# hardcamls/video-coding

Measured on NVIDIA B200. Metric: decoded megapixels/sec (1920x1080 420 baseline), higher is better.
Workload: dtype u8/int16/int32 (integer, bit-exact)

## Files before the change

### video-coding_b200/csrc/hcj_common.h

```cpp
#pragma once
#include <stdint.h>

#define HCJ_LUT_BITS 10
#define HCJ_LUT_SIZE (1 << HCJ_LUT_BITS)
#define HCJ_LUT_NSUB 8
#define HCJ_LUT_SUB_BITS 6
#define HCJ_LUT_SUB_SIZE (1 << HCJ_LUT_SUB_BITS)
#define HCJ_LUT_ENTRIES (HCJ_LUT_SIZE + HCJ_LUT_NSUB * HCJ_LUT_SUB_SIZE)
#define HCJ_MAX_BPM 10
#define HCJ_MAX_COMP 4
#ifndef HCJ_IDCT_THREADS
#define HCJ_IDCT_THREADS 128
#endif
#ifndef HCJ_IDCT_CTAS_PER_SM
#define HCJ_IDCT_CTAS_PER_SM 5
#endif

#define HCJ_DEV_OK 0
#define HCJ_DEV_NO_DC_CODE (-2)
#define HCJ_DEV_NO_AC_CODE (-3)
#define HCJ_DEV_COEF_INDEX (-4)
#define HCJ_DEV_BITS_OOB (-9)
#define HCJ_DEV_NO_TERMINATOR (-20)
#define HCJ_DEV_RESTART_COUNT (-21)
#define HCJ_DEV_DC_RANGE (-23)

struct HcjTableMeta {
  uint32_t full_off;
  uint32_t max_bits;
};

struct HcjTableSet {
  HcjTableMeta meta[HCJ_MAX_COMP][2];
  uint32_t primary_off;
  uint32_t npairs;
};

struct HcjCompGeom {
  int32_t hs, vs;
  int32_t decoded_w, decoded_h;
  int32_t actual_w, actual_h;
  int32_t pair;
  int32_t qt;
  int32_t first_blk;
  uint8_t up_h, up_v;
  uint16_t pad_;
  uint64_t plane_off;
  uint64_t out_off;
};

struct HcjImageDesc {
  uint64_t file_off;
  uint32_t file_len;
  uint32_t scan_start;
  uint64_t ent_off;
  uint32_t ent_cap;
  uint32_t seg_off;
  uint32_t nseg_expected;
  uint32_t ri;
  int32_t ncomp, bpm;
  int32_t mcus_wide, mcus_high;
  uint32_t nmcu, nblocks;
  uint64_t coef_off;
  HcjCompGeom comp[HCJ_MAX_COMP];
  uint8_t blk_comp[HCJ_MAX_BPM + 2];
  uint8_t blk_bx[HCJ_MAX_BPM + 2];
  uint8_t blk_by[HCJ_MAX_BPM + 2];
  uint8_t wide_idct;
// ... 25 lines not shown
```

### video-coding_b200/csrc/hcj_device.cuh

```cuda
#pragma once
#include <stdint.h>

#include "hcj_common.h"

#if defined(__CUDACC__)
#define HCJ_HD __host__ __device__ __forceinline__
#else
#define HCJ_HD inline
#endif

namespace hcjdev {

HCJ_HD uint32_t bswap32(uint32_t x) {
#if defined(__CUDA_ARCH__)
  return __byte_perm(x, 0, 0x0123);
#else
  return (x >> 24) | ((x >> 8) & 0xff00u) | ((x << 8) & 0xff0000u) | (x << 24);
#endif
}

HCJ_HD uint32_t load_raw_word(const uint32_t *__restrict__ words, uint32_t idx, uint32_t end_bits) {
  if ((idx << 5) >= end_bits) return 0u;
#if defined(__CUDA_ARCH__)
  return __ldg(words + idx);
// ... 347 lines not shown
    }
  }
  if (err) *err_pos = br.pos;
  return err;
}

struct FastReader {
  const uint32_t *words;
  uint32_t pos, w0, w1, r0, r1;
  HCJ_HD static uint32_t ld(const uint32_t *p) {
#if defined(__CUDA_ARCH__)
    return __ldg(p);
#else
    return *p;
#endif
  }
  HCJ_HD void init(const uint32_t *words_, uint32_t pos_) {
    words = words_;
    pos = pos_;
    const uint32_t i = pos_ >> 5;
    w0 = bswap32(ld(words + i));
    w1 = bswap32(ld(words + i + 1));
    r0 = ld(words + i + 2);
    r1 = ld(words + i + 3);
  }
  HCJ_HD uint32_t window() const {
#if defined(__CUDA_ARCH__)
    return __funnelshift_l(w1, w0, pos);
#else
    uint32_t s = pos & 31u;
    return s ? (w0 << s) | (w1 >> (32u - s)) : w0;
#endif
  }
  HCJ_HD void consume(uint32_t n) {
    const uint32_t np = pos + n;
    const uint32_t cross = (np ^ pos) & 32u;
    pos = np;
    if (cross) {
      w0 = w1;
      w1 = bswap32(r0);
      r0 = r1;
    }
#if defined(__CUDA_ARCH__)
    asm volatile(
        "{\n\t.reg .pred p;\n\tsetp.ne.u32 p, %2, 0;\n\t@p ld.global.nc.L2::128B.u32 %0, [%1];\n\t}"
        : "+r"(r1)
        : "l"(words + (np >> 5) + 3), "r"(cross));
#else
    if (cross) r1 = ld(words + (np >> 5) + 3);
#endif
  }
};

HCJ_HD int32_t fast_value(uint32_t win, uint32_t len, uint32_t sh) {
  const uint32_t t = win << len;
  const uint32_t m = shr_clamp(t, sh), mask = shr_clamp(0xffffffffu, sh);
  return (int32_t)m - (int32_t)(mask & ~(uint32_t)((int32_t)t >> 31));
}

HCJ_HD bool z_block_done(uint32_t z) { return z >= 64u; }
HCJ_HD bool z_overrun(uint32_t z) { return z > 64u && z <= HCJ_ZADV_EOB; }
HCJ_HD bool z_no_code(uint32_t z) { return z >= 256u; }

struct ExactLane {
  FastReader br;
  uint32_t c, z;
  uint32_t tdc, tac, qoff;
  uint32_t comp;
  int32_t blk;
  int32_t pcur, p0, p1, p2, p3;
  uint32_t share, sumabs, qmax;
};

HCJ_HD void exact_bind_block(ExactLane &s, const FastTables T) {
  const BlkInfo bi = T.blkinfo[s.c];
  s.tdc = bi.tdc;
  s.tac = bi.tac;
  s.qoff = bi.qoff;
  s.comp = bi.comp_qmax & 0xffu;
  s.qmax = bi.comp_qmax >> 8;
  s.pcur = s.comp == 0u ? s.p0 : s.comp == 1u ? s.p1 : s.comp == 2u ? s.p2 : s.p3;
}
HCJ_HD void exact_save_pred(ExactLane &s) {
  s.p0 = s.comp == 0u ? s.pcur : s.p0;
  s.p1 = s.comp == 1u ? s.pcur : s.p1;
  s.p2 = s.comp == 2u ? s.pcur : s.p2;
  s.p3 = s.comp == 3u ? s.pcur : s.p3;
}
HCJ_HD void exact_next_block(ExactLane &s, const FastTables T, uint32_t bpm) {
  exact_save_pred(s);
  s.c = s.c + 1u == bpm ? 0u : s.c + 1u;
  s.z = 0u;
  s.share = 0u;
  s.sumabs = 0u;
  exact_bind_block(s, T);
}
HCJ_HD bool exact_share_may_be_wide(const ExactLane &s) {
  return s.sumabs >= 0x10000u || (uint64_t)s.share + (uint64_t)s.sumabs * s.qmax >= (uint64_t)HCJ_WIDE_SHARE;
}
HCJ_HD uint32_t exact_share(const ExactLane &s, const FastTables T, const int16_t *row) {
  uint64_t a = s.share;
  for (int zi = 1; zi < 64; zi++) {
    const int32_t v = row[zi];
    a += (uint64_t)(uint32_t)(v < 0 ? -v : v) * (uint32_t)T.quant[s.qoff + zi];
  }
  return a > 0xffffffffull ? 0xffffffffu : (uint32_t)a;
}

HCJ_HD void exact_ac_step(ExactLane &s, const FastTables T, int16_t *row) {
  const uint32_t win = s.br.window();
  const uint32_t e = fast_lookup(T, s.tac, win, false);
  const uint32_t znext = s.z + (e >> 24);
  const uint32_t sh = byte_of(e, 2);
  const int32_t v = fast_value(win, byte_of(e, 1), sh);
  if (sh != 32u && znext <= 64u) {
    row[znext - 1u] = (int16_t)v;
    s.sumabs += (uint32_t)(v < 0 ? -v : v);
  }
  s.br.consume(byte_of(e, 0));
  s.z = znext;
}
HCJ_HD void exact_ac_undo_no_code(ExactLane &s) { s.z -= 255u; }

HCJ_HD bool exact_dc_step(ExactLane &s, const FastTables T, int16_t *row) {
  const uint32_t win = s.br.window();
  const uint32_t e = fast_lookup(T, s.tdc, win, true);
  const int32_t pc = s.pcur + fast_value(win, byte_of(e, 1), byte_of(e, 2));
  if (e == HCJ_FAST_NONE || pc < -32768 || pc > 32767) return false;
  s.pcur = pc;
  s.blk++;
  row[0] = (int16_t)pc;
  s.share = (uint32_t)(pc < 0 ? -pc : pc) * (uint32_t)T.quant[s.qoff];
  s.sumabs = 0u;
  s.br.consume(byte_of(e, 0));
  s.z = 1u;
  return true;
}

HCJ_HD uint32_t multi_sync_entry(const uint32_t *fast_ac , uint32_t idx) {
  const uint32_t e = fast_ac[idx];
  if (e & HCJ_FAST_SLOW) return e;
  uint32_t pos = e & 0xffu, pre = 0, adv = e >> 24;
  while (adv != HCJ_ZADV_EOB && pos < (uint32_t)HCJ_LUT_BITS && pre + adv < 63u) {
    const uint32_t e2 = fast_ac[(idx << pos) & (HCJ_LUT_SIZE - 1)];
    if (e2 & HCJ_FAST_SLOW) break;
    if (pos + ((e2 >> 8) & 0xffu) > (uint32_t)HCJ_LUT_BITS) break;
    if (pos + (e2 & 0xffu) > 31u) break;
    pre += adv;
    adv = e2 >> 24;
    pos += e2 & 0xffu;
  }
  const uint32_t tot = pre + adv > 127u ? 127u : pre + adv;
  return pos | (pre << 8) | (tot << 24);
}

struct SyncLane {
  FastReader br;
  uint32_t c, z;
  uint32_t tdc, tac, comp;
  uint32_t nstart;
  int32_t d0, d1, d2, d3;
  uint32_t first_p, nbefore;
};
HCJ_HD void sync_bind_block(SyncLane &s, const FastTables T) {
  const BlkInfo bi = T.blkinfo[s.c];
  s.tdc = bi.tdc;
  s.tac = bi.tac;
  s.comp = bi.comp_qmax & 0xffu;
}
HCJ_HD void sync_next_block(SyncLane &s, const FastTables T, uint32_t bpm) {
  s.c = s.c + 1u == bpm ? 0u : s.c + 1u;
  s.z = 0u;
  sync_bind_block(s, T);
}
HCJ_HD void sync_ac_step_multi(SyncLane &s, const FastTables T, uint32_t lim_m) {
  const uint32_t win = s.br.window();
  const uint32_t idx = win >> (32 - HCJ_LUT_BITS);
// ... 132 lines not shown
  constexpr int t[64] = {0,  1,  8,  16, 9,  2,  3,  10, 17, 24, 32, 25, 18, 11, 4,  5,  12, 19, 26, 33, 40, 48,
                         41, 34, 27, 20, 13, 6,  7,  14, 21, 28, 35, 42, 49, 56, 57, 50, 43, 36, 29, 22, 15, 23,
                         30, 37, 44, 51, 58, 59, 52, 45, 38, 31, 39, 46, 53, 60, 61, 54, 47, 55, 62, 63};
  return t[i];
}
HCJ_HD constexpr int zigzag_forward(int i) {
  constexpr int t[64] = {0,  1,  5,  6,  14, 15, 27, 28, 2,  4,  7,  13, 16, 26, 29, 42, 3,  8,  12, 17, 25, 30,
                         41, 43, 9,  11, 18, 24, 31, 40, 44, 53, 10, 19, 23, 32, 39, 45, 52, 54, 20, 22, 33, 38,
                         46, 51, 55, 60, 21, 34, 37, 47, 50, 56, 59, 61, 35, 36, 48, 49, 57, 58, 62, 63};
  return t[i];
}

#define HCJ_QD(i, q) (((i) & 1) ? (int32_t)(q) << 8 : (int32_t)(q))
HCJ_HD int32_t dequant_lo(uint32_t cw, int32_t q) {
#if defined(__CUDA_ARCH__)
  int32_t d;
  asm("dp2a.lo.s32.u32 %0, %1, %2, %3;" : "=r"(d) : "r"(cw), "r"(q), "r"(0));
  return d;
#else
  return (int32_t)(int16_t)(cw & 0xffffu) * q;
#endif
}
HCJ_HD int32_t dequant_hi(uint32_t cw, int32_t q) {
#if defined(__CUDA_ARCH__)
  int32_t d;
  asm("dp2a.lo.s32.u32 %0, %1, %2, %3;" : "=r"(d) : "r"(cw), "r"(q), "r"(0));
  return d;
#else
  return (int32_t)(int16_t)(cw >> 16) * (q >> 8);
#endif
}

template <bool GUARD = true>
HCJ_HD bool reconstruct_fast(const uint32_t cw[32], const int32_t *__restrict__ qd , uint32_t out[16]) {
  int32_t v[64];
  uint32_t l1 = 0;
#pragma unroll
  for (int j = 0; j < 32; j++) {
    int32_t d0 = dequant_lo(cw[j], qd[2 * j]), d1 = dequant_hi(cw[j], qd[2 * j + 1]);
    v[zigzag_inverse(2 * j)] = d0;
    v[zigzag_inverse(2 * j + 1)] = d1;
    if (GUARD) l1 += (uint32_t)(d0 < 0 ? -d0 : d0) + (uint32_t)(d1 < 0 ? -d1 : d1);
  }
  if (GUARD && l1 >= (uint32_t)HCJ_IDCT_L1_LIMIT) return false;
  idct_8x8<int32_t, (128 << 14)>(v);
#pragma unroll
  for (int r = 0; r < 8; r++) {
    out[2 * r] = pack4_sat(v[8 * r], v[8 * r + 1], v[8 * r + 2], v[8 * r + 3]);
    out[2 * r + 1] = pack4_sat(v[8 * r + 4], v[8 * r + 5], v[8 * r + 6], v[8 * r + 7]);
  }
  return true;
}

HCJ_HD void reconstruct_wide(const uint32_t *cw, const int32_t *q, uint32_t *out) {
  int64_t w[64];
  for (int j = 0; j < 32; j++) {
    int64_t lo = (int16_t)(cw[j] & 0xffffu), hi = (int16_t)(cw[j] >> 16);
    w[zigzag_inverse(2 * j)] = lo * (int64_t)q[2 * j];
    w[zigzag_inverse(2 * j + 1)] = hi * (int64_t)q[2 * j + 1];
  }
  idct_8x8<int64_t>(w);
  for (int k = 0; k < 16; k++) {
    uint32_t word = 0;
    for (int i = 0; i < 4; i++) {
      int64_t sv = w[4 * k + i] < -128 ? -128 : w[4 * k + i] > 127 ? 127 : w[4 * k + i];
      word |= (uint32_t)(sv + 128) << (8 * i);
    }
    out[k] = word;
  }
}

HCJ_HD void reconstruct_block(const int16_t c[64], const uint16_t q[64], bool force_wide, uint8_t pix[64]) {
  uint32_t cw[32], out[16];
  int32_t q32[64], qd[64];
  for (int j = 0; j < 32; j++) cw[j] = (uint32_t)(uint16_t)c[2 * j] | ((uint32_t)(uint16_t)c[2 * j + 1] << 16);
  for (int i = 0; i < 64; i++) {
    q32[i] = q[i];
    qd[i] = HCJ_QD(i, q[i]);
  }
  if (force_wide || !reconstruct_fast<true>(cw, qd, out)) reconstruct_wide(cw, q32, out);
  for (int k = 0; k < 64; k++) pix[k] = (uint8_t)(out[k >> 2] >> (8 * (k & 3)));
}

template <typename T>
HCJ_HD T dequant_nat(const uint32_t cw[32], const int32_t *q, int n) {
  const int z = zigzag_forward(n);
  const int32_t c = (z & 1) ? (int32_t)(int16_t)(cw[z >> 1] >> 16) : (int32_t)(int16_t)(cw[z >> 1] & 0xffffu);
  return (T)c * (T)q[z];
}

template <typename T>
HCJ_HD void idct4_pass(T c0, T c1, T c2, T c3, T c5, T c6, T c7, int sh, T o[4]) {
  const T t0 = c0 * (T)(1 << 14);
  const T t2 = c2 * (T)15137 - c6 * (T)6270;
  const T t10 = t0 + t2, t12 = t0 - t2;
  const T a0 = c1 * (T)8697 - c3 * (T)17799 + c5 * (T)11893 - c7 * (T)1730;
  const T a2 = c1 * (T)20995 + c3 * (T)7373 - c5 * (T)4926 - c7 * (T)4176;
  const T r = (T)1 << (sh - 1);
  o[0] = (t10 + a2 + r) >> sh;
  o[1] = (t12 + a0 + r) >> sh;
  o[2] = (t12 - a0 + r) >> sh;
  o[3] = (t10 - a2 + r) >> sh;
}

template <typename T>
HCJ_HD void idct2_pass(T c0, T c1, T c3, T c5, T c7, int sh, T o[2]) {
// ... 362 lines not shown
```

### video-coding_b200/csrc/hcj_kernels.cu

```cuda
#include <cuda.h>
#include <cuda_runtime.h>
#include <stdint.h>
#include <stdlib.h>

#include "hcj_device.cuh"
#include "hcj_kernels.cuh"

namespace hcjk {

using namespace hcjdev;

constexpr int DS_THREADS = 256;
constexpr uint32_t DS_TILE = DS_THREADS * 16;

__device__ __forceinline__ uint32_t warp_incl_scan(uint32_t v, int lane) {
#pragma unroll
  for (int d = 1; d < 32; d <<= 1) {
    uint32_t t = __shfl_up_sync(0xffffffffu, v, d);
    if (lane >= d) v += t;
  }
  return v;
}

struct DsClass {
// ... 553 lines not shown
    sc.total_bits = total_bits;
    sc.bpm = d.bpm;
    sc.wide_flags = b.wide_flags;
    sc.blk_base = d.coef_off;
  }
  if (threadIdx.x < (uint32_t)d.ncomp) sc.tab[threadIdx.x] = tables_of(st, threadIdx.x);
}

__device__ __forceinline__ void raise_status(HcjImageState *st, int code, uint32_t bit_pos) {
  atomicMin(&st->err_key, ((unsigned long long)bit_pos << 8) | (unsigned long long)(-code));
}

constexpr int HR_ROW_WORDS = 36;
constexpr int HR_STAGE_WORDS = 32 * HR_ROW_WORDS;

struct PassIn {
  uint32_t p, cz, hi, end_bits;
  int32_t blk;
  int32_t pred[HCJ_MAX_COMP];
  int32_t nblocks_end;
  uint32_t share;
  bool valid;
};

__device__ __forceinline__ void warp_store_full(uint32_t mask, int32_t blk, uint32_t *stage, int lane, int16_t *coefs) {
  const int quarter = lane >> 3, sub = lane & 7;
#pragma unroll
  for (int p = 0; p < 8; p++) {
    if (((mask >> (4 * p)) & 0xfu) == 0u) continue;
    const int l = 4 * p + quarter;
    const int32_t bidx = __shfl_sync(0xffffffffu, blk, l);
    if ((mask >> l) & 1u) {
      uint4 *src = reinterpret_cast<uint4 *>(stage + l * HR_ROW_WORDS) + sub;
      const uint4 v = *src;
      *src = make_uint4(0u, 0u, 0u, 0u);
      reinterpret_cast<uint4 *>(coefs + (size_t)bidx * 64)[sub] = v;
    }
  }
}

__device__ __forceinline__ int warp_exact_fast(const ScanCtx &sc, const FastTables T, uint32_t *stage, int lane, PassIn &in,
                                               int16_t *coefs, uint32_t *err_pos) {
  const uint32_t bpm = sc.bpm;
  int16_t *row = reinterpret_cast<int16_t *>(stage + lane * HR_ROW_WORDS);
  const uint32_t lim = in.end_bits >= 32u ? in.end_bits - 32u : 0u;
  ExactLane s;
  s.c = in.cz >> 8;
  s.z = in.cz & 0xffu;
  s.blk = in.blk;
  s.p0 = in.pred[0], s.p1 = in.pred[1], s.p2 = in.pred[2], s.p3 = in.pred[3];
  s.share = in.share;
  s.sumabs = 0u;
  const bool entered = in.valid && in.p < lim;
  s.br.init(sc.words, entered ? in.p : 0u);
  exact_bind_block(s, T);
  int st = !entered ? 2 : s.z != 0u ? 0 : 1;
  int err = HCJ_DEV_OK;

  for (;;) {
    while (__any_sync(0xffffffffu, st == 0)) {
#pragma unroll
      for (int u = 0; u < 2; u++) {
        if (st == 0) {
          if (s.br.pos >= lim) {
            st = 2;
          } else {
            exact_ac_step(s, T, row);
            st = z_block_done(s.z) ? 1 : 0;
          }
        }
      }
    }
    if (!__any_sync(0xffffffffu, st == 1)) break;
    {
      if (st == 1 && s.z > 64u) {
        if (z_no_code(s.z)) {
          exact_ac_undo_no_code(s);
          st = 2;
        } else if (z_overrun(s.z)) {
          err = HCJ_DEV_COEF_INDEX;
          *err_pos = s.br.pos;
          st = 3;
        }
      }
      const bool have = st == 1 && s.z != 0u;
      if (have && exact_share_may_be_wide(s) && exact_share(s, T, row) >= (uint32_t)HCJ_WIDE_SHARE) flag_wide_block(sc, s.blk);
      warp_store_full(__ballot_sync(0xffffffffu, have), s.blk, stage, lane, coefs);
      if (have) exact_next_block(s, T, bpm);
      if (st == 1) {
        if (s.blk + 1 >= in.nblocks_end || s.br.pos >= lim || (s.c == 0u && s.br.pos >= in.hi)) st = 2;
        else st = exact_dc_step(s, T, row) ? 0 : 2;
      }
    }
  }
  if (entered && st == 2 && s.z != 0u) s.share = exact_share(s, T, row);
  if (entered) {
    exact_save_pred(s);
    in.p = s.br.pos;
    in.cz = (s.c << 8) | s.z;
    in.blk = s.blk;
    in.pred[0] = s.p0, in.pred[1] = s.p1, in.pred[2] = s.p2, in.pred[3] = s.p3;
    in.share = s.share;
    if (err) {
      in.valid = false;
      uint4 *src = reinterpret_cast<uint4 *>(row);
#pragma unroll
      for (int j = 0; j < 8; j++) src[j] = make_uint4(0u, 0u, 0u, 0u);
    }
  }
  return err;
}

__device__ __forceinline__ int warp_exact_pass(const ScanCtx &sc, const SmemTables &st, const Local L, uint32_t *stage,
                                               int lane, const PassIn &in, int16_t *coefs, uint32_t *err_pos) {
  uint32_t *coefs32 = reinterpret_cast<uint32_t *>(coefs);
  const uint32_t bpm = sc.bpm;
  uint32_t c = in.cz >> 8, z = in.cz & 0xffu, share = in.share;
  int32_t blk = in.blk;
  bool active = in.valid;
  uint32_t comp = st.blk_comp[c];
  Tables t = sc.tab[comp];
  const uint32_t stage_sa = (uint32_t)__cvta_generic_to_shared(stage);
  const uint32_t mine_sa = stage_sa + (uint32_t)lane * HR_ROW_WORDS * 4u;
  const uint32_t quant_sa = (uint32_t)__cvta_generic_to_shared(st.quant);
  uint32_t q_sa = quant_sa + comp * 512u;
  int32_t p0 = in.pred[0], p1 = in.pred[1], p2 = in.pred[2], p3 = in.pred[3];
  int32_t pcur = comp == 0u ? p0 : comp == 1u ? p1 : comp == 2u ? p2 : p3;
// ... 566 lines not shown
  fill_scan_ctx(sc, st, b, d, si.state->ent_len * 8u);
  __syncthreads();
  const Local LT{T, st.quant, st.blk_comp};
  int16_t *coefs = b.coefs + d.coef_off * 64;

  const uint32_t j = blockIdx.x * SPEC_WRITE_THREADS + threadIdx.x;
  PassIn in;
  in.valid = j < si.nsub;
  const uint32_t jj = in.valid ? j : 0u;
  const SpecSub q = spec_sub(si, jj);
  const uint32_t first = si.first[jj];
  in.valid = in.valid && (first >> 31) == 0u;
  in.p = q.lo + (first & 0xffffu);
  in.cz = 0u;
  const int4 dc = si.dc[jj], dpre = si.dpre[jj];
  in.pred[0] = dc.x + dpre.x, in.pred[1] = dc.y + dpre.y, in.pred[2] = dc.z + dpre.z, in.pred[3] = dc.w + dpre.w;
  in.blk = si.blk[jj] + (int32_t)((first >> 16) & 15u) - 1;
  in.hi = q.hi;
  in.end_bits = q.uend;
  in.nblocks_end = q.blk_end;
  in.share = 0;
  uint32_t err_pos = 0;
  int err = warp_exact_fast(sc, T, stage, lane, in, coefs, &err_pos);
  if (err) raise_status(si.state, err, err_pos);
  err = warp_exact_pass(sc, st, LT, stage, lane, in, coefs, &err_pos);
  if (err) raise_status(si.state, err, err_pos);
}

static inline size_t spec_base_smem(const DecodeBatchDev &b) {
  return ((sizeof(SmemTables) + 15) & ~size_t(15)) + ((sizeof(ScanCtx) + 15) & ~size_t(15)) + lut_smem_bytes(b);
}
void launch_huff_spec(const DecodeBatchDev &b, cudaStream_t s) {
  if (b.ls_hi <= b.ls_lo || b.max_sub_chunks == 0) return;
  const size_t base = spec_base_smem(b);
  const size_t smem_sync = base + multi_smem_bytes(b);
  const size_t smem_write = base + (SPEC_WRITE_THREADS / 32) * HR_STAGE_WORDS * sizeof(uint32_t);
  const dim3 grid(b.max_sub_chunks, b.ls_hi - b.ls_lo);
  if (b.spec_has_units) k_spec_units<<<b.ls_hi - b.ls_lo, SPEC_THREADS, 0, s>>>(b);
  k_spec_sync<<<grid, SPEC_THREADS, smem_sync, s>>>(b);
  k_spec_fix<<<b.ls_hi - b.ls_lo, SPEC_FIX_THREADS, base, s>>>(b);
  const dim3 grid_w((b.max_sub_chunks * SPEC_THREADS + SPEC_WRITE_THREADS - 1) / SPEC_WRITE_THREADS, b.ls_hi - b.ls_lo);
  k_spec_write<<<grid_w, SPEC_WRITE_THREADS, smem_write, s>>>(b);
}
int huff_spec_kernel_count(const DecodeBatchDev &b) { return 3 + (b.spec_has_units ? 1 : 0); }

constexpr int IDCT_MAX_THREADS = HCJ_IDCT_THREADS;

__device__ __forceinline__ void cp_async16(void *smem, const void *gmem) {
  uint32_t sa = (uint32_t)__cvta_generic_to_shared(smem);
  asm volatile("cp.async.cg.shared.global [%0], [%1], 16;\n" ::"r"(sa), "l"(gmem) : "memory");
}
__device__ __forceinline__ void cp_async_wait_all() { asm volatile("cp.async.wait_all;\n" ::: "memory"); }

__device__ __forceinline__ void store_block_rows(const uint32_t pix[16], uint8_t *dst, int stride, int x, int y,
                                                 int w_limit, int h_limit) {
  uint8_t *row = dst + (size_t)y * stride + x;
  const bool fast = (x + 8 <= w_limit) && (((uintptr_t)row & 7u) == 0) && ((stride & 7) == 0);
  if (fast) {
#pragma unroll
    for (int r = 0; r < 8; r++)
      if (y + r < h_limit) *reinterpret_cast<uint2 *>(row + (size_t)r * stride) = make_uint2(pix[2 * r], pix[2 * r + 1]);
  } else {
#pragma unroll
    for (int r = 0; r < 8; r++) {
      if (y + r >= h_limit) break;
#pragma unroll
      for (int i = 0; i < 8; i++)
        if (x + i < w_limit) row[(size_t)r * stride + i] = (uint8_t)(pix[2 * r + (i >> 2)] >> (8 * (i & 3)));
    }
  }
}

__device__ __noinline__ void wide_block_store(const uint32_t *cw, const int32_t *q, uint8_t *dst, int stride, int x, int y,
                                              int w_limit, int h_limit) {
  uint32_t pix[16];
  reconstruct_wide(cw, q, pix);
  store_block_rows(pix, dst, stride, x, y, w_limit, h_limit);
}

__device__ __noinline__ void wide_block_store_staged(const uint4 *tile, int slot, const int32_t *q, uint8_t *dst, int stride, int x,
                                                     int y, int w_limit, int h_limit) {
  uint32_t cw[32], pix[16];
  for (int j = 0; j < 8; j++) {
    const uint4 u = tile[slot * 8 + (j ^ (slot & 7))];
    cw[4 * j] = u.x, cw[4 * j + 1] = u.y, cw[4 * j + 2] = u.z, cw[4 * j + 3] = u.w;
  }
  reconstruct_wide(cw, q, pix);
  store_block_rows(pix, dst, stride, x, y, w_limit, h_limit);
}

template <int K>
__device__ __forceinline__ void store_block_rows_k(const uint32_t *pix, uint8_t *dst, int stride, int x, int y, int w_limit,
                                                   int h_limit) {
  uint8_t *row = dst + (size_t)y * stride + x;
  const bool fast = (x + K <= w_limit) && (((uintptr_t)row & (K - 1)) == 0) && ((stride & (K - 1)) == 0);
#pragma unroll
  for (int r = 0; r < K; r++) {
    if (y + r >= h_limit) break;
    uint8_t *p = row + (size_t)r * stride;
    if (fast) {
      if (K == 4) *reinterpret_cast<uint32_t *>(p) = pix[r];
      else if (K == 2) *reinterpret_cast<uint16_t *>(p) = (uint16_t)pix[r];
      else *p = (uint8_t)pix[r];
    } else {
#pragma unroll
      for (int i = 0; i < K; i++)
        if (x + i < w_limit) p[i] = (uint8_t)(pix[r] >> (8 * i));
    }
  }
}

template <int K>
__device__ __noinline__ void scaled_block_store_wide(const uint4 *tile, int slot, const int32_t *q, uint8_t *dst, int stride, int x,
                                                     int y, int h_limit) {
  uint32_t cw[32], pix[K];
  for (int j = 0; j < 8; j++) {
    const uint4 u = tile[slot * 8 + (j ^ (slot & 7))];
// ... 356 lines not shown
  const int tm = t.tm, vs_log = d.comp[0].vs == 2 ? 1 : 0;
  const int rows = 8 << vs_log, pitch_l = 16 * tm, pitch_c = 8 * tm;
  uint8_t *xcb = xch + rows * pitch_l, *xcr = xcb + 8 * pitch_c;
  const int x = (int)t.m0 * (int)((mp.misc >> 12) & 63u) + (int)(mp.xy & 0xffffu);
  const int y = (int)t.my * (int)((mp.misc >> 18) & 63u) + (int)(mp.xy >> 16);
  uint8_t *dst = c == 0 ? xch + (mp.xy >> 16) * pitch_l + (mp.xy & 0xffffu) : (c == 1 ? xcb : xcr) + (mp.xy & 0xffffu);
  const int pitch = c == 0 ? pitch_l : pitch_c;
  {
    uint32_t pix[16];
    reconstruct_fast<false>(cw, st.q + c * 128 + 64, pix);
    if (mine && !wide) {
#pragma unroll
      for (int r = 0; r < 8; r++) *reinterpret_cast<uint2 *>(dst + r * pitch) = make_uint2(pix[2 * r], pix[2 * r + 1]);
      if (c != 0) store_block_rows(pix, mp.plane, mp.stride, x, y, mp.stride, mp.h_limit);
    }
  }
  if (any_wide && wide) {
    const int16_t *cb = b.coefs + (t.blk0 + (uint64_t)slot) * 64;
    wide_block_to_xch(cb, st.q + c * 128, dst, pitch);
    if (c != 0) wide_block_store(reinterpret_cast<const uint32_t *>(cb), st.q + c * 128, mp.plane, mp.stride, x, y, mp.stride, mp.h_limit);
  }
  __syncthreads();
  const int width = d.width, height = d.height, cwid = d.comp[1].actual_w, chh = d.comp[1].actual_h;
  const int x_tile = (int)t.m0 * 16, y_tile = (int)t.my * rows, cx_tile = (int)t.m0 * 8, cy_tile = (int)t.my * 8;
  const bool right_deferred = cx_tile + 8 * tm < cwid;
  const bool bottom_deferred = vs_log && cy_tile + 8 < chh;
  uint8_t *out = b.out + d.out_off;
  uint8_t *plane_y = b.planes + d.comp[0].plane_off;
  const int stride_y = d.comp[0].decoded_w;
  const int nunits = rows * tm, nhalf = vs_log ? 8 * tm : nunits;
  const uint32_t recip = 65536u / (uint32_t)tm + 1u;
  for (int idx = tid; idx < nunits; idx += IDCT_MAX_THREADS) {
    const int k = idx < nhalf ? idx : idx - nhalf;
    const int rk = (int)(((uint32_t)k * recip) >> 16), m = k - rk * tm;
    const int r = vs_log ? 2 * rk + (idx < nhalf ? 0 : 1) : rk;
    const int px = x_tile + 16 * m, py = y_tile + r;
    if (py >= height || px >= width) continue;
    const uint4 vy = *reinterpret_cast<const uint4 *>(xch + r * pitch_l + 16 * m);
    if ((right_deferred && m == tm - 1) || (bottom_deferred && r == rows - 1)) {
      *reinterpret_cast<uint4 *>(plane_y + (size_t)py * stride_y + px) = vy;
      continue;
    }
    const int crow = r >> vs_log;
    const bool oy = vs_log && (r & 1);
    const int crow1 = (oy && cy_tile + crow + 1 <= chh - 1) ? crow + 1 : crow;
    const int nvalid = cwid - (cx_tile + 8 * m);
    uint32_t o[12];
    sub_unit16_to_rgb(vy, xcb + crow * pitch_c + 8 * m, xcb + crow1 * pitch_c + 8 * m, xcr + crow * pitch_c + 8 * m,
                      xcr + crow1 * pitch_c + 8 * m, nvalid, oy, o);
    store_any<12>(out + ((size_t)py * width + px) * 3, o, 3 * min(16, width - px));
  }
}

template <bool FUSED, int K = 8, bool ISLOW = false>
__global__ void __launch_bounds__(IDCT_MAX_THREADS, HCJ_IDCT_CTAS_PER_SM)
    k_idct_persistent(const __grid_constant__ DecodeBatchDev b, int mode) {
  extern __shared__ uint4 s_dyn[];
  IdctStage *stages = reinterpret_cast<IdctStage *>(reinterpret_cast<uint8_t *>(s_dyn) + ((1024u - (smem_u32(s_dyn) & 1023u)) & 1023u));
  const int tid = threadIdx.x;
  const uint32_t total = b.tile_hi - b.tile_lo;
  const uint32_t chunk = (total + gridDim.x - 1) / gridDim.x;
  const uint32_t begin = b.tile_lo + min(blockIdx.x * chunk, total), end = b.tile_lo + min((blockIdx.x + 1) * chunk, total);
  if (begin >= end) return;

  __shared__ IdctTile s_ring[IDCT_RING];
  __shared__ IdctMapSmem s_map;
  if (tid == 0) {
    mbar_init(&stages[0].full, 1);
    mbar_init(&stages[1].full, 1);
    asm volatile("fence.mbarrier_init.release.cluster;" ::: "memory");
    idct_fetch_record(b, s_ring, begin, end);
    idct_fetch_record(b, s_ring, begin + 1, end);
    idct_fetch_record(b, s_ring, begin + 2, end);
    asm volatile("cp.async.wait_group 1;\n" ::: "memory");
    idct_issue(b, s_ring[begin % IDCT_RING], stages[0]);
  }
  __syncthreads();
  for (uint32_t id = begin; id < end; id++) {
    const int buf = (int)(id - begin) & 1;
    IdctStage &st = stages[buf];
    if (tid == 0) {
      idct_fetch_record(b, s_ring, id + 3, end);
      if (id + 1 < end) idct_issue(b, s_ring[(id + 1) % IDCT_RING], stages[buf ^ 1]);
    }
    const IdctTile &t = s_ring[id % IDCT_RING];
    if (t.remap || id == begin) {
      const HcjImageDesc &d = b.descs[t.img];
      const int tm = t.tm;
      int rem = tid, c = 0;
      for (; c < d.ncomp - 1; c++) {
        int n = tm * d.comp[c].hs * d.comp[c].vs;
        if (rem < n) break;
        rem -= n;
      }
      const HcjCompGeom &g = d.comp[c];
      const int rowlen = tm * g.hs;
      const int by = (rem >= rowlen) + (rem >= 2 * rowlen) + (rem >= 3 * rowlen);
      const int r2 = rem - by * rowlen;
      const int m = g.hs == 1 ? r2 : g.hs == 2 ? r2 >> 1 : g.hs == 4 ? r2 >> 2 : r2 / 3;
      const int bx = r2 - m * g.hs;
      const uint32_t slot = (uint32_t)(m * d.bpm + g.first_blk + by * g.hs + bx);
      const bool mine = tid < (int)t.nblk;
      IdctMap mp;
      mp.xy = (uint32_t)(m * g.hs * K + bx * K) | (uint32_t)(by * K) << 16;
      mp.misc = (mine ? slot : 0u) | (uint32_t)c << 8 | (mine ? 1u << 10 : 0u) | (d.wide_idct ? 1u << 11 : 0u) |
                (uint32_t)(g.hs * K) << 12 | (uint32_t)(g.vs * K) << 18;
      if (mode == 0) {
        mp.plane = b.out + d.out_off + g.out_off;
        mp.stride = g.actual_w;
        mp.h_limit = g.actual_h;
      } else {
        mp.plane = (mode == 2 ? b.planes : b.out + d.out_off) + g.plane_off;
        mp.stride = g.decoded_w;
        mp.h_limit = g.decoded_h;
      }
      s_map.put(tid, mp);
    }
    mbar_wait(&st.full, (uint32_t)((id - begin) >> 1) & 1u);
    int tnow;
    asm volatile("mov.u32 %0, %%tid.x;" : "=r"(tnow));
    const IdctMap mp = s_map.get(tnow);
    if (FUSED && t.fused == 1u) {
      idct_tile_rgb444(b, t, st, mp, tnow);
    } else if (FUSED && t.fused == 2u) {
      idct_tile_rgb_sub(b, t, st, mp, tnow);
    } else if ((K != 8 || ISLOW) && (mp.misc & (1u << 10))) {
      const int slot = (int)(mp.misc & 255u);
      const uint32_t fbit = (uint32_t)(t.blk0 & 127u) + slot;
      const bool wide = (mp.misc & (1u << 11)) || ((reinterpret_cast<const uint32_t *>(st.flags)[fbit >> 5] >> (fbit & 31u)) & 1u);
      const int x = (int)t.m0 * (int)((mp.misc >> 12) & 63u) + (int)(mp.xy & 0xffffu);
      const int y = (int)t.my * (int)((mp.misc >> 18) & 63u) + (int)(mp.xy >> 16);
      if (ISLOW) islow_block_store(st.tile, slot, st.q + ((mp.misc >> 8) & 3u) * 128u, wide, mp.plane, mp.stride, x, y, mp.h_limit);
      else scaled_block_store<K>(st.tile, slot, st.q + ((mp.misc >> 8) & 3u) * 128u, wide, mp.plane, mp.stride, x, y, mp.h_limit);
    } else if (K == 8 && (mp.misc & (1u << 10))) {
      const int slot = (int)(mp.misc & 255u);
      uint32_t cw[32];
#pragma unroll
      for (int j = 0; j < 8; j++) {
        uint4 u = st.tile[slot * 8 + (j ^ (slot & 7))];
        cw[4 * j] = u.x;
        cw[4 * j + 1] = u.y;
        cw[4 * j + 2] = u.z;
        cw[4 * j + 3] = u.w;
      }
      const uint32_t fbit = (uint32_t)(t.blk0 & 127u) + slot;
      const bool wide = (mp.misc & (1u << 11)) || ((reinterpret_cast<const uint32_t *>(st.flags)[fbit >> 5] >> (fbit & 31u)) & 1u);
      const int x = (int)t.m0 * (int)((mp.misc >> 12) & 63u) + (int)(mp.xy & 0xffffu);
      const int y = (int)t.my * (int)((mp.misc >> 18) & 63u) + (int)(mp.xy >> 16);
      const int32_t *q = st.q + ((mp.misc >> 8) & 3u) * 128u;
      if (wide) {
        wide_block_store_staged(st.tile, slot, q, mp.plane, mp.stride, x, y, mp.stride, mp.h_limit);
      } else {
        uint32_t pix[16];
        reconstruct_fast<false>(cw, q + 64, pix);
        store_block_rows(pix, mp.plane, mp.stride, x, y, mp.stride, mp.h_limit);
      }
    }
    if (tid == 0) asm volatile("cp.async.wait_group 1;\n" ::: "memory");
    __syncthreads();
  }
}

constexpr size_t IDCT_SMEM = 2 * sizeof(IdctStage) + 1024;

void launch_idct(const DecodeBatchDev &b, int mode, cudaStream_t s) {
  if (b.img_hi <= b.img_lo || b.tile_hi <= b.tile_lo) return;
  const int grid = HCJ_IDCT_CTAS_PER_SM * (b.sm_count > 0 ? b.sm_count : 148);
  k_idct_plan<<<dim3((b.max_idct_tiles + 127) / 128, b.img_hi - b.img_lo), 128, 0, s>>>(b);
  const uint32_t total = b.tile_hi - b.tile_lo;
  const unsigned ctas = (unsigned)(total < (uint32_t)grid ? total : grid);
  if (b.islow) k_idct_persistent<false, 8, true><<<ctas, IDCT_MAX_THREADS, IDCT_SMEM, s>>>(b, mode);
  else if (b.block_k == 4) k_idct_persistent<false, 4><<<ctas, IDCT_MAX_THREADS, IDCT_SMEM, s>>>(b, mode);
  else if (b.block_k == 2) k_idct_persistent<false, 2><<<ctas, IDCT_MAX_THREADS, IDCT_SMEM, s>>>(b, mode);
  else if (b.block_k == 1) k_idct_persistent<false, 1><<<ctas, IDCT_MAX_THREADS, IDCT_SMEM, s>>>(b, mode);
  else if (mode == 2 && (b.has_fused || b.has_fused_sub)) k_idct_persistent<true><<<ctas, IDCT_MAX_THREADS, IDCT_SMEM, s>>>(b, mode);
  else k_idct_persistent<false><<<ctas, IDCT_MAX_THREADS, IDCT_SMEM, s>>>(b, mode);
}

int make_coef_tensor_map(DecodeBatchDev *b) {
  typedef CUresult (*EncodeTiled)(CUtensorMap *, CUtensorMapDataType, cuuint32_t, void *, const cuuint64_t *, const cuuint64_t *,
                                  const cuuint32_t *, const cuuint32_t *, CUtensorMapInterleave, CUtensorMapSwizzle,
                                  CUtensorMapL2promotion, CUtensorMapFloatOOBfill);
  static EncodeTiled encode = nullptr;
  if (!encode) {
    void *fn = nullptr;
    cudaDriverEntryPointQueryResult q;
    cudaError_t e = cudaGetDriverEntryPoint("cuTensorMapEncodeTiled", &fn, cudaEnableDefault, &q);
    if (e != cudaSuccess) return (int)e;
    if (q != cudaDriverEntryPointSuccess || !fn) return (int)cudaErrorNotSupported;
    encode = reinterpret_cast<EncodeTiled>(fn);
  }
  static_assert(sizeof(CUtensorMap) == sizeof(b->coef_map), "CUtensorMap is 128 bytes");
  const cuuint64_t dims[2] = {64, b->total_blocks ? b->total_blocks : 1};
  const cuuint64_t strides[1] = {128};
  const cuuint32_t box[2] = {64, IDCT_MAX_THREADS};
  const cuuint32_t estr[2] = {1, 1};
  CUresult r = encode(reinterpret_cast<CUtensorMap *>(b->coef_map), CU_TENSOR_MAP_DATA_TYPE_UINT16, 2, b->coefs, dims, strides, box,
                      estr, CU_TENSOR_MAP_INTERLEAVE_NONE, CU_TENSOR_MAP_SWIZZLE_128B, CU_TENSOR_MAP_L2_PROMOTION_L2_128B,
                      CU_TENSOR_MAP_FLOAT_OOB_FILL_NONE);
  return r == CUDA_SUCCESS ? 0 : (int)cudaErrorInvalidValue;
}

__global__ void k_idct_blocks(const int16_t *coefs, size_t nblocks, const uint16_t *qt, int force_wide, uint8_t *out) {
  __shared__ int32_t s_q[128];
  if (threadIdx.x < 64) {
    s_q[threadIdx.x] = qt[threadIdx.x];
    s_q[64 + threadIdx.x] = HCJ_QD(threadIdx.x, qt[threadIdx.x]);
  }
  __syncthreads();
  size_t i = (size_t)blockIdx.x * blockDim.x + threadIdx.x;
  if (i >= nblocks) return;
  uint32_t cw[32], pix[16];
  const uint4 *src = reinterpret_cast<const uint4 *>(coefs + i * 64);
#pragma unroll
  for (int j = 0; j < 8; j++) {
    uint4 u = __ldg(src + j);
    cw[4 * j] = u.x;
    cw[4 * j + 1] = u.y;
    cw[4 * j + 2] = u.z;
    cw[4 * j + 3] = u.w;
  }
  if (force_wide || !reconstruct_fast<true>(cw, s_q + 64, pix)) {
    wide_block_store(reinterpret_cast<const uint32_t *>(coefs + i * 64), s_q, out + i * 64, 8, 0, 0, 8, 8);
    return;
  }
  uint4 *dst = reinterpret_cast<uint4 *>(out + i * 64);
#pragma unroll
  for (int j = 0; j < 4; j++) dst[j] = make_uint4(pix[4 * j], pix[4 * j + 1], pix[4 * j + 2], pix[4 * j + 3]);
}
// ... 590 lines not shown
```

Baseline: 430,200.

## Split each 8x8 IDCT block across two threads exchanging halves via shared memory

For the common non-fused 8x8 path, each block is now handled by a pair of threads in a 256-thread CTA. Each thread computes four IDCT rows, the pair swaps halves through the tile's shared-memory slot using named 64-thread barriers, and each thread then does four columns and stores four output rows. This is meant to halve per-thread register pressure and serial work and raise parallelism. In exchange it adds extra shared-memory traffic and barriers, and it lowers CTAs per SM to 4.

```diff
diff --git a/video-coding_b200/csrc/hcj_common.h b/video-coding_b200/csrc/hcj_common.h
--- a/video-coding_b200/csrc/hcj_common.h
+++ b/video-coding_b200/csrc/hcj_common.h
@@ -14,6 +14,9 @@
 #endif
 #ifndef HCJ_IDCT_CTAS_PER_SM
 #define HCJ_IDCT_CTAS_PER_SM 5
+#endif
+#ifndef HCJ_IDCT_PAIR_CTAS_PER_SM
+#define HCJ_IDCT_PAIR_CTAS_PER_SM 4
 #endif
 
 #define HCJ_DEV_OK 0
diff --git a/video-coding_b200/csrc/hcj_device.cuh b/video-coding_b200/csrc/hcj_device.cuh
--- a/video-coding_b200/csrc/hcj_device.cuh
+++ b/video-coding_b200/csrc/hcj_device.cuh
@@ -732,6 +732,29 @@
   return true;
 }
 
+template <int H>
+HCJ_HD void idct_row_part(const uint32_t cw[32], const int32_t *__restrict__ qd , int r, int32_t keep[4], int32_t send[4]) {
+  int32_t v[8];
+#pragma unroll
+  for (int c = 0; c < 8; c++) {
+    const int z = zigzag_forward(8 * (4 * H + r) + c);
+    v[c] = (z & 1) ? dequant_hi(cw[z >> 1], qd[z]) : dequant_lo(cw[z >> 1], qd[z]);
+  }
+  idct_row<int32_t, 1>(v);
+#pragma unroll
+  for (int c = 0; c < 4; c++) keep[c] = v[4 * H + c], send[c] = v[4 * (1 - H) + c];
+}
+template <int H>
+HCJ_HD void idct_cols_part(const int32_t keep[16], const int32_t recv[16], uint32_t out[8]) {
+  int32_t v[32];
+#pragma unroll
+  for (int i = 0; i < 16; i++) v[16 * H + i] = keep[i], v[16 * (1 - H) + i] = recv[i];
+#pragma unroll
+  for (int c = 0; c < 4; c++) idct_col<int32_t, 4, (128 << 14)>(v + c);
+#pragma unroll
+  for (int r = 0; r < 8; r++) out[r] = pack4_sat(v[4 * r], v[4 * r + 1], v[4 * r + 2], v[4 * r + 3]);
+}
+
 HCJ_HD void reconstruct_wide(const uint32_t *cw, const int32_t *q, uint32_t *out) {
   int64_t w[64];
   for (int j = 0; j < 32; j++) {
diff --git a/video-coding_b200/csrc/hcj_kernels.cu b/video-coding_b200/csrc/hcj_kernels.cu
--- a/video-coding_b200/csrc/hcj_kernels.cu
+++ b/video-coding_b200/csrc/hcj_kernels.cu
@@ -1322,17 +1322,18 @@
 }
 __device__ __forceinline__ void cp_async_wait_all() { asm volatile("cp.async.wait_all;\n" ::: "memory"); }
 
-__device__ __forceinline__ void store_block_rows(const uint32_t pix[16], uint8_t *dst, int stride, int x, int y,
+template <int ROWS = 8>
+__device__ __forceinline__ void store_block_rows(const uint32_t pix[2 * ROWS], uint8_t *dst, int stride, int x, int y,
                                                  int w_limit, int h_limit) {
   uint8_t *row = dst + (size_t)y * stride + x;
   const bool fast = (x + 8 <= w_limit) && (((uintptr_t)row & 7u) == 0) && ((stride & 7) == 0);
   if (fast) {
 #pragma unroll
-    for (int r = 0; r < 8; r++)
+    for (int r = 0; r < ROWS; r++)
       if (y + r < h_limit) *reinterpret_cast<uint2 *>(row + (size_t)r * stride) = make_uint2(pix[2 * r], pix[2 * r + 1]);
   } else {
 #pragma unroll
-    for (int r = 0; r < 8; r++) {
+    for (int r = 0; r < ROWS; r++) {
       if (y + r >= h_limit) break;
 #pragma unroll
       for (int i = 0; i < 8; i++)
@@ -1795,12 +1796,63 @@
   }
 }
 
-template <bool FUSED, int K = 8, bool ISLOW = false>
-__global__ void __launch_bounds__(IDCT_MAX_THREADS, HCJ_IDCT_CTAS_PER_SM)
+constexpr int IDCT_PAIR_THREADS = 2 * IDCT_MAX_THREADS;
+
+__device__ __forceinline__ void pair_sync(int pair) { asm volatile("bar.sync %0, 64;" ::"r"(pair + 1) : "memory"); }
+
+template <int H>
+__device__ __forceinline__ void idct_block_part(const DecodeBatchDev &b, IdctStage &st, const IdctTile &t, const IdctMap &mp, int pair) {
+  const bool mine = (mp.misc & (1u << 10)) != 0u;
+  const int slot = (int)(mp.misc & 255u), sw = slot & 7;
+  uint4 *blk = st.tile + slot * 8;
+  const uint32_t fbit = (uint32_t)(t.blk0 & 127u) + slot;
+  const bool wide = (mp.misc & (1u << 11)) || ((reinterpret_cast<const uint32_t *>(st.flags)[fbit >> 5] >> (fbit & 31u)) & 1u);
+  const int x = (int)t.m0 * (int)((mp.misc >> 12) & 63u) + (int)(mp.xy & 0xffffu);
+  const int y = (int)t.my * (int)((mp.misc >> 18) & 63u) + (int)(mp.xy >> 16);
+  const int32_t *q = st.q + ((mp.misc >> 8) & 3u) * 128u;
+  uint32_t cw[32];
+#pragma unroll
+  for (int j = 0; j < 8; j++) {
+    const uint4 u = blk[j ^ sw];
+    cw[4 * j] = u.x, cw[4 * j + 1] = u.y, cw[4 * j + 2] = u.z, cw[4 * j + 3] = u.w;
+  }
+  pair_sync(pair);
+  int32_t keep[16], xch[16];
+#pragma unroll
+  for (int r = 0; r < 4; r++) {
+    idct_row_part<H>(cw, q + 64, r, keep + 4 * r, xch + 4 * r);
+    if (mine) blk[(4 * H + r) ^ sw] = make_uint4(xch[4 * r], xch[4 * r + 1], xch[4 * r + 2], xch[4 * r + 3]);
+  }
+  pair_sync(pair);
+#pragma unroll
+  for (int k = 0; k < 4; k++) {
+    const uint4 u = blk[(4 * (1 - H) + k) ^ sw];
+    xch[4 * k] = (int32_t)u.x, xch[4 * k + 1] = (int32_t)u.y, xch[4 * k + 2] = (int32_t)u.z, xch[4 * k + 3] = (int32_t)u.w;
+  }
+  uint32_t out[8];
+  idct_cols_part<H>(keep, xch, out);
+  if (mine) {
+    blk[(4 * (1 - H)) ^ sw] = make_uint4(out[4 * (1 - H)], out[4 * (1 - H) + 1], out[4 * (1 - H) + 2], out[4 * (1 - H) + 3]);
+    asm volatile("fence.proxy.async.shared::cta;" ::: "memory");
+  }
+  pair_sync(pair);
+  const uint4 o = blk[(4 * H) ^ sw];
+  if (mine && !wide) {
+    const uint32_t pix[8] = {H ? o.x : out[0], H ? out[4] : o.x, H ? o.y : out[1], H ? out[5] : o.y,
+                             H ? o.z : out[2], H ? out[6] : o.z, H ? o.w : out[3], H ? out[7] : o.w};
+    store_block_rows<4>(pix, mp.plane, mp.stride, x, y + 4 * H, mp.stride, mp.h_limit);
+  }
+  if (H == 0 && mine && wide)
+    wide_block_store(reinterpret_cast<const uint32_t *>(b.coefs + (t.blk0 + (uint64_t)slot) * 64), q, mp.plane, mp.stride, x, y, mp.stride, mp.h_limit);
+}
+
+template <bool FUSED, int K = 8, bool ISLOW = false, bool PAIR = !FUSED && K == 8 && !ISLOW>
+__global__ void __launch_bounds__(PAIR ? IDCT_PAIR_THREADS : IDCT_MAX_THREADS, PAIR ? HCJ_IDCT_PAIR_CTAS_PER_SM : HCJ_IDCT_CTAS_PER_SM)
     k_idct_persistent(const __grid_constant__ DecodeBatchDev b, int mode) {
   extern __shared__ uint4 s_dyn[];
   IdctStage *stages = reinterpret_cast<IdctStage *>(reinterpret_cast<uint8_t *>(s_dyn) + ((1024u - (smem_u32(s_dyn) & 1023u)) & 1023u));
   const int tid = threadIdx.x;
+  const int blk = PAIR ? (tid >> 6) * 32 + (tid & 31) : tid;
   const uint32_t total = b.tile_hi - b.tile_lo;
   const uint32_t chunk = (total + gridDim.x - 1) / gridDim.x;
   const uint32_t begin = b.tile_lo + min(blockIdx.x * chunk, total), end = b.tile_lo + min((blockIdx.x + 1) * chunk, total);
@@ -1830,7 +1882,7 @@
     if (t.remap || id == begin) {
       const HcjImageDesc &d = b.descs[t.img];
       const int tm = t.tm;
-      int rem = tid, c = 0;
+      int rem = blk, c = 0;
       for (; c < d.ncomp - 1; c++) {
         int n = tm * d.comp[c].hs * d.comp[c].vs;
         if (rem < n) break;
@@ -1843,7 +1895,7 @@
       const int m = g.hs == 1 ? r2 : g.hs == 2 ? r2 >> 1 : g.hs == 4 ? r2 >> 2 : r2 / 3;
       const int bx = r2 - m * g.hs;
       const uint32_t slot = (uint32_t)(m * d.bpm + g.first_blk + by * g.hs + bx);
-      const bool mine = tid < (int)t.nblk;
+      const bool mine = blk < (int)t.nblk;
       IdctMap mp;
       mp.xy = (uint32_t)(m * g.hs * K + bx * K) | (uint32_t)(by * K) << 16;
       mp.misc = (mine ? slot : 0u) | (uint32_t)c << 8 | (mine ? 1u << 10 : 0u) | (d.wide_idct ? 1u << 11 : 0u) |
@@ -1857,13 +1909,17 @@
         mp.stride = g.decoded_w;
         mp.h_limit = g.decoded_h;
       }
-      s_map.put(tid, mp);
+      if (!PAIR || !(tid & 32)) s_map.put(blk, mp);
+      if (PAIR) pair_sync(tid >> 6);
     }
     mbar_wait(&st.full, (uint32_t)((id - begin) >> 1) & 1u);
     int tnow;
     asm volatile("mov.u32 %0, %%tid.x;" : "=r"(tnow));
-    const IdctMap mp = s_map.get(tnow);
-    if (FUSED && t.fused == 1u) {
+    const IdctMap mp = s_map.get(PAIR ? (tnow >> 6) * 32 + (tnow & 31) : tnow);
+    if (PAIR) {
+      if (tnow & 32) idct_block_part<1>(b, st, t, mp, tnow >> 6);
+      else idct_block_part<0>(b, st, t, mp, tnow >> 6);
+    } else if (FUSED && t.fused == 1u) {
       idct_tile_rgb444(b, t, st, mp, tnow);
     } else if (FUSED && t.fused == 2u) {
       idct_tile_rgb_sub(b, t, st, mp, tnow);
@@ -1908,16 +1964,16 @@
 
 void launch_idct(const DecodeBatchDev &b, int mode, cudaStream_t s) {
   if (b.img_hi <= b.img_lo || b.tile_hi <= b.tile_lo) return;
-  const int grid = HCJ_IDCT_CTAS_PER_SM * (b.sm_count > 0 ? b.sm_count : 148);
   k_idct_plan<<<dim3((b.max_idct_tiles + 127) / 128, b.img_hi - b.img_lo), 128, 0, s>>>(b);
   const uint32_t total = b.tile_hi - b.tile_lo;
-  const unsigned ctas = (unsigned)(total < (uint32_t)grid ? total : grid);
+  const uint32_t sms = b.sm_count > 0 ? (uint32_t)b.sm_count : 148u;
+  const unsigned ctas = (unsigned)min(total, HCJ_IDCT_CTAS_PER_SM * sms), pair_ctas = (unsigned)min(total, HCJ_IDCT_PAIR_CTAS_PER_SM * sms);
   if (b.islow) k_idct_persistent<false, 8, true><<<ctas, IDCT_MAX_THREADS, IDCT_SMEM, s>>>(b, mode);
   else if (b.block_k == 4) k_idct_persistent<false, 4><<<ctas, IDCT_MAX_THREADS, IDCT_SMEM, s>>>(b, mode);
   else if (b.block_k == 2) k_idct_persistent<false, 2><<<ctas, IDCT_MAX_THREADS, IDCT_SMEM, s>>>(b, mode);
   else if (b.block_k == 1) k_idct_persistent<false, 1><<<ctas, IDCT_MAX_THREADS, IDCT_SMEM, s>>>(b, mode);
   else if (mode == 2 && (b.has_fused || b.has_fused_sub)) k_idct_persistent<true><<<ctas, IDCT_MAX_THREADS, IDCT_SMEM, s>>>(b, mode);
-  else k_idct_persistent<false><<<ctas, IDCT_MAX_THREADS, IDCT_SMEM, s>>>(b, mode);
+  else k_idct_persistent<false><<<pair_ctas, IDCT_PAIR_THREADS, IDCT_SMEM, s>>>(b, mode);
 }
 
 int make_coef_tensor_map(DecodeBatchDev *b) {
```

Measured after the change: 388,800 (median of 6 runs). 9.6% lower.

## Replace per-word bit reader with prefetching 8-word queue reader in exact decode

Applied to the files above, without the earlier changes.

Swaps the FastReader in the exact per-lane Huffman decoder for a QueueReader that holds an 8-word register queue and issues 128-bit predicated vector prefetches of the next four words. Refills happen at warp-synchronous points, with a new 'needs refill' state that pauses lanes whose queue runs low. The goal is to hide global-load latency and replace per-crossing scalar loads with fewer wide loads. In exchange it raises register pressure through the queue array and the select-based refill, and it can add extra warp loop iterations when lanes stall for a refill.

```diff
diff --git a/video-coding_b200/csrc/hcj_device.cuh b/video-coding_b200/csrc/hcj_device.cuh
--- a/video-coding_b200/csrc/hcj_device.cuh
+++ b/video-coding_b200/csrc/hcj_device.cuh
@@ -423,6 +423,76 @@
   }
 };
 
+struct QueueReader {
+  const uint32_t *words;
+  uint32_t pos;
+  uint32_t q[8];
+  uint32_t tail;
+  uint32_t lim;
+  uint32_t pn0, pn1, pn2, pn3;
+  const uint32_t *pnext;
+
+  HCJ_HD void request() {
+#if defined(__CUDA_ARCH__)
+    asm volatile(
+        "{\n\t.reg .pred p;\n\tsetp.ne.u64 p, %4, 0;\n\t@p ld.global.nc.L2::128B.v4.u32 {%0, %1, %2, %3}, [%4];\n\t}"
+        : "+r"(pn0), "+r"(pn1), "+r"(pn2), "+r"(pn3)
+        : "l"(pnext));
+#else
+    if (pnext) pn0 = pnext[0], pn1 = pnext[1], pn2 = pnext[2], pn3 = pnext[3];
+#endif
+    pnext = nullptr;
+  }
+  HCJ_HD void set_next(const uint32_t *words, uint32_t end_bits) { pnext = (tail << 5) < end_bits ? words + tail : nullptr; }
+  HCJ_HD void set_lim(uint32_t end_bits) {
+    const uint32_t dlim = end_bits >= 32u ? end_bits - 32u : 0u;
+    const uint32_t qlim = (tail - 1u) << 5;
+    lim = dlim < qlim ? dlim : qlim;
+  }
+  HCJ_HD void init(const uint32_t *words_, uint32_t pos_, uint32_t end_bits = 0xffffffffu) {
+    words = words_;
+    pos = pos_;
+    const uint32_t i = pos_ >> 5;
+#pragma unroll
+    for (int k = 0; k < 8; k++) q[k] = bswap32(load_raw_word(words, i + k, end_bits));
+    tail = (i & ~3u) + 8u;
+    pn0 = pn1 = pn2 = pn3 = 0u;
+    set_next(words, end_bits);
+    set_lim(end_bits);
+  }
+  HCJ_HD uint32_t window() const {
+#if defined(__CUDA_ARCH__)
+    return __funnelshift_l(q[1], q[0], pos);
+#else
+    uint32_t s = pos & 31u;
+    return s ? (q[0] << s) | (q[1] >> (32u - s)) : q[0];
+#endif
+  }
+  HCJ_HD void consume(uint32_t n) {
+    const uint32_t np = pos + n;
+    const bool cross = ((np ^ pos) & 32u) != 0u;
+    pos = np;
+    if (cross) {
+#pragma unroll
+      for (int k = 0; k < 7; k++) q[k] = q[k + 1];
+    }
+  }
+  HCJ_HD void refill(const uint32_t *words, uint32_t end_bits) {
+    const uint32_t n = tail - (pos >> 5);
+    if (n <= 4u && (tail << 5) < end_bits && pnext == nullptr) {
+      const uint32_t p[4] = {bswap32(pn0), bswap32(pn1), bswap32(pn2), bswap32(pn3)};
+#pragma unroll
+      for (int k = 1; k < 8; k++)
+#pragma unroll
+        for (int j = 0; j < 4; j++)
+          if (k - j >= 1 && k - j <= 4 && n == (uint32_t)(k - j)) q[k] = p[j];
+      tail += 4u;
+      set_next(words, end_bits);
+    }
+    set_lim(end_bits);
+  }
+};
+
 HCJ_HD int32_t fast_value(uint32_t win, uint32_t len, uint32_t sh) {
   const uint32_t t = win << len;
   const uint32_t m = shr_clamp(t, sh), mask = shr_clamp(0xffffffffu, sh);
@@ -434,7 +504,7 @@
 HCJ_HD bool z_no_code(uint32_t z) { return z >= 256u; }
 
 struct ExactLane {
-  FastReader br;
+  QueueReader br;
   uint32_t c, z;
   uint32_t tdc, tac, qoff;
   uint32_t comp;
@@ -478,7 +548,16 @@
   return a > 0xffffffffull ? 0xffffffffu : (uint32_t)a;
 }
 
+HCJ_HD void exact_refill_on_host(ExactLane &s) {
+#if !defined(__CUDA_ARCH__)
+  if (s.br.pos >= s.br.lim) {
+    s.br.request();
+    s.br.refill(s.br.words, 0xffffffffu);
+  }
+#endif
+}
 HCJ_HD void exact_ac_step(ExactLane &s, const FastTables T, int16_t *row) {
+  exact_refill_on_host(s);
   const uint32_t win = s.br.window();
   const uint32_t e = fast_lookup(T, s.tac, win, false);
   const uint32_t znext = s.z + (e >> 24);
@@ -494,6 +573,7 @@
 HCJ_HD void exact_ac_undo_no_code(ExactLane &s) { s.z -= 255u; }
 
 HCJ_HD bool exact_dc_step(ExactLane &s, const FastTables T, int16_t *row) {
+  exact_refill_on_host(s);
   const uint32_t win = s.br.window();
   const uint32_t e = fast_lookup(T, s.tdc, win, true);
   const int32_t pc = s.pcur + fast_value(win, byte_of(e, 1), byte_of(e, 2));
diff --git a/video-coding_b200/csrc/hcj_kernels.cu b/video-coding_b200/csrc/hcj_kernels.cu
--- a/video-coding_b200/csrc/hcj_kernels.cu
+++ b/video-coding_b200/csrc/hcj_kernels.cu
@@ -629,7 +629,7 @@
   s.share = in.share;
   s.sumabs = 0u;
   const bool entered = in.valid && in.p < lim;
-  s.br.init(sc.words, entered ? in.p : 0u);
+  s.br.init(sc.words, entered ? in.p : 0u, entered ? in.end_bits : 0u);
   exact_bind_block(s, T);
   int st = !entered ? 2 : s.z != 0u ? 0 : 1;
   int err = HCJ_DEV_OK;
@@ -639,17 +639,20 @@
 #pragma unroll
       for (int u = 0; u < 2; u++) {
         if (st == 0) {
-          if (s.br.pos >= lim) {
-            st = 2;
+          if (s.br.pos >= s.br.lim) {
+            st = 4;
           } else {
+            if (u == 0) s.br.request();
             exact_ac_step(s, T, row);
             st = z_block_done(s.z) ? 1 : 0;
           }
         }
       }
     }
-    if (!__any_sync(0xffffffffu, st == 1)) break;
+    if (!__any_sync(0xffffffffu, st == 1 || st == 4)) break;
     {
+      if (st == 4) st = s.br.pos >= lim ? 2 : 0;
+      if (st == 0 || st == 1) s.br.refill(sc.words, in.end_bits);
       if (st == 1 && s.z > 64u) {
         if (z_no_code(s.z)) {
           exact_ac_undo_no_code(s);
```

Measured after the change: 430,700 before, 405,200 after, median of 6. 5.9% lower.
